# ReillyBova/Global-Illumination

Hardware: AMD Instinct MI355X
Metric: Mpixel-samples/sec (and ms/frame) at 1024^2 aa=2, 1M+1M photons (higher is better)
Workload: dtype f64 (shading/geometry), f32 (photon positions)

## Files before the change

### global-illumination_amd/csrc/gi_host.cpp

```cpp
#include <hip/hip_runtime.h>
#include <dlfcn.h>
#include <rccl/rccl.h>
#include <algorithm>
#include <cfloat>
#include <chrono>
#include <cmath>
#include <cstdio>
#include <cstdlib>
#include <cstring>
#include <functional>
#include <mutex>
#include <string>
#include <thread>
#include <vector>
#include "../../include/gi.h"
#include "gi_denoise.h"
#include "gi_radiance.h"
#include "gi_kdbuild.h"
#include "gi_kernels.h"
#include "gi_scene.h"
#include "gi_sort.h"

using namespace gi;

// ... 262 lines not shown
  DBuf d_nodes, d_elems, d_shapes, d_tris, d_bvh, d_mats, d_lights, d_lut, d_stats;
  HostMap hmap[2];
  DevMap dmap[2];
  bool map_valid[2] = {false, false};
  int leaf_size[2] = {64, 256};
  bool gpu_kd = true;
  KdBuildScratch kdb;
  DBuf kd_ph;
  int wave_cap_mul = 1;
  int chunk_cap_big = 512;
  bool chunk_dk_exact = true;
  int chunk_minsub_big = 64;
  int chunk_minsub = 32;
  double fb_ms[2] = {0, 0};
  uint64_t fb_q[2] = {0, 0};
  double p2_ms[2] = {0, 0};
  uint64_t p2_q[2] = {0, 0};
  int last_kind[2] = {-1, -1};
  bool knn_log = false;
  int knn_dbg = 0;
  int render_dbg = 0;
  int64_t slot_limit = 0;
  int elem_pretest = -1;
  gi_progress_fn progress = nullptr;
  void *progress_user = nullptr;
  int64_t progress_done = 0, progress_total = 0;
  int sel_slack = 64;
  int knn_qpl = 1;
  DBuf ind_cont, ind_ncont;
  DBuf mc_cont, mc_ncont;
  DBuf mc_cont2, mc_ncont2;
  bool mc_sub = true;
  int mc_persist = -1;
  DBuf prim_rgb;
  DBuf d_rays, d_ray_ids;
  std::vector<gi_ray> ray_stage;
  std::vector<uint64_t> id_stage;
  DBuf ind_tab, mc_tab;
  DBuf ind_trows, ind_rows;
  DBuf ind_masks;
  bool split_ind = true;
  double ind_frac = 0.25;
  DBuf spawn, npaths, path_off, nmc, mc_off, nind, ind_off, base, pixels, rgbf, rgb8, qcount, stats_bak;
  DBuf qpos[2], qshade[2], qkey[2], qout[2];
  bool chunk_big2 = true;
  int chunk_cap_big2 = 1024;
  int chunk_cap_big3 = 0;
  bool chunk_lane2 = true;
  int chunk_minsub_big2 = 64;
  bool chunk_dk = true;
  bool chunk_fb_all = false;
  int knn_general_mode = 0;
  int key_bits[2] = {10, 16};
  bool row_order = true;
  bool surf_key = true;
  bool surf_key_c = true;
  bool fb_wave = true;
  bool use_dk = true;
  DBuf qseg[2];
  size_t qcap_hint[2] = {0, 0};
  KeySortScratch keysort[2];
  int knn_kernel_kind = -1;
  DBuf scan_lvl[8], scan_out[8];
  DBuf pcounts, poffs, pbuf;
  DBuf pkeys, pcursor, ptmp;
  DBuf pacc, pglob;
// ... 918 lines not shown
    HIPCHK(c, c->ind_trows.ensure((size_t)(ntiles + 1) * 4));
    HIPCHK(c, c->ind_rows.ensure((size_t)(ntiles + 1) * 4));
    launch_ind_tiles(a.nind, nprim, c->ind_trows.as<uint32_t>(), c->stream);
    HIPCHK(c, launch_scan(c->ind_trows.as<uint32_t>(), c->ind_rows.as<uint32_t>(), ntiles, t, c->stream));
    uint32_t trows = 0;
    HIPCHK(c, hipMemcpyAsync(&trows, c->ind_rows.as<uint32_t>() + ntiles, 4, hipMemcpyDeviceToHost,
                             c->stream));
    HIPCHK(c, hipStreamSynchronize(c->stream));
    const uint64_t tind = 64ull * trows;
    if ((uint64_t)total_paths + tind + (uint64_t)nprim > slot_limit) {
      if (npix == 1)
        return fail(c, GI_ERR_ALLOC, "one output pixel's samples need more than 2^32 path slots");
      HIPCHK(c, hipMemcpyAsync(c->d_stats.p, c->stats_bak.p, ST_BYTES, hipMemcpyDeviceToDevice,
                               c->stream));
      HIPCHK(c, hipStreamSynchronize(c->stream));
      shrink *= 2;
      c->batch_reruns++;
      npix = 0;
      continue;
    }
    a.ind_rows = c->ind_rows.as<uint32_t>();
    a.ind_g0 = total_paths;
    a.tind = (int64_t)tind;
    HIPCHK(c, c->ind_tab.ensure(((size_t)trows + 1) * 8));
    launch_ind_row_tile(a.ind_rows, ntiles, c->ind_tab.as<uint64_t>(), c->stream);
    a.ind_row_info = c->ind_tab.as<uint64_t>();
    HIPCHK(c, c->ind_masks.ensure(((size_t)trows + 1) * 16));
    a.ind_qmask = c->ind_masks.as<uint64_t>();
    a.ind_bmask = a.ind_qmask + trows + 1;
    HIPCHK(c, c->base.ensure(((size_t)total_paths + tind) * 24));
    a.base = c->base.as<double>();
    const uint64_t ind_full = 64 * ((((uint64_t)a.tind + 63) / 64 + IND_QS - 1) / IND_QS);
    if (a.split_ind && a.total_ind > 0) HIPCHK(c, c->ind_ncont.ensure(IND_QS * 32 * 4));
    if (a.split_ind && a.total_mc > 0 && a.F.indirect) {
      const uint64_t full = 64 * ((((uint64_t)a.total_mc + 63) / 64 + IND_QS - 1) / IND_QS);
      HIPCHK(c, c->mc_cont.ensure((size_t)IND_QS * full * sizeof(IndCont)));
      HIPCHK(c, c->mc_ncont.ensure(IND_QS * 32 * 4));
      a.mc_cont = c->mc_cont.as<IndCont>();
      a.mc_ncont = c->mc_ncont.as<uint32_t>();
      a.mc_cap_s = (uint32_t)full;
      if (c->mc_persist > 0 || (c->mc_persist < 0 && !a.S.hard_lights)) {
        a.mc_next = c->qcount.as<uint32_t>() + 2;
        a.mc_persist_blocks = c->mc_persist > 0 ? c->mc_persist : 1024;
      }
      if (c->mc_sub) {
        HIPCHK(c, c->mc_cont2.ensure((size_t)IND_QS * full * sizeof(IndCont)));
        HIPCHK(c, c->mc_ncont2.ensure(IND_QS * 32 * 4));
        a.mc_cont2 = c->mc_cont2.as<IndCont>();
        a.mc_ncont2 = c->mc_ncont2.as<uint32_t>();
      }
    }
    uint32_t nq[2] = {0, 0};
    HIPCHK(c, hipMemcpyAsync(c->stats_bak.p, c->d_stats.p, ST_BYTES,
                             hipMemcpyDeviceToDevice, c->stream));
    uint32_t qbase[2] = {(uint32_t)(nprim + tind), (uint32_t)nprim};
    a.qind_base = nprim;
    a.tiled_skip = c->row_order && c->key_bits[0] <= 10 && !P.irradiance_cache && a.ind_qmask &&
                   (a.total_ind > 0 || tind == 0);
    for (int attempt = 0; attempt < 3; attempt++) {
      for (int l = 0; l < 2; l++) {
        size_t cap = std::max<size_t>(c->qcap_hint[l], (size_t)qbase[l] + 1024);
        if (attempt == 0) {
          const double per_mc = std::max(2.0, c->mc_app_rate[l]);
          size_t pred = (size_t)qbase[l] + (size_t)(1.25 * per_mc * (double)a.total_mc) + 1024;
          cap = std::max(cap, std::min<size_t>(pred, 0xFFFFFFF0u));
        }
        HIPCHK(c, c->qpos[l].ensure(cap * 16));
        HIPCHK(c, c->qshade[l].ensure(cap * sizeof(QShade)));
        HIPCHK(c, c->qkey[l].ensure(cap * 8));
        a.qpos[l] = c->qpos[l].as<float4>();
        a.qshade[l] = c->qshade[l].as<QShade>();
        a.qkey[l] = c->qkey[l].as<uint64_t>();
        a.qcap[l] = (uint32_t)std::min<size_t>(cap, 0xFFFFFFF0u);
      }
      if (a.split_ind && a.total_ind > 0) {
        uint64_t cap_s = std::min<uint64_t>(ind_full, 64 * ((uint64_t)(ind_full * c->ind_frac) / 64 + 1));
        HIPCHK(c, c->ind_cont.ensure((size_t)IND_QS * cap_s * sizeof(IndCont)));
        a.ind_cap_s = (uint32_t)cap_s;
        a.ind_cont = c->ind_cont.as<IndCont>();
        a.ind_ncont = c->ind_ncont.as<uint32_t>();
      }
      a.qcount = c->qcount.as<uint32_t>();
      HIPCHK(c, hipMemcpyAsync(c->qcount.p, qbase, 8, hipMemcpyHostToDevice, c->stream));
      if (!a.tiled_skip && tind > (uint64_t)a.total_ind) launch_ind_pad(a, c->stream);
      launch_path(a, c->stream, c->stream2, c->ev_fork, c->ev_join, true);
      HIPCHK(c, hipGetLastError());
      HIPCHK(c, hipMemcpyAsync(nq, c->qcount.p, 8, hipMemcpyDeviceToHost, c->stream));
      uint32_t fills[IND_QS * 32];
      if (a.split_ind && a.total_ind > 0)
        HIPCHK(c, hipMemcpyAsync(fills, c->ind_ncont.p, sizeof fills, hipMemcpyDeviceToHost, c->stream));
      HIPCHK(c, hipStreamSynchronize(c->stream));
      attempts_used = attempt + 1;
      bool ok = nq[0] <= a.qcap[0] && nq[1] <= a.qcap[1];
      if (a.split_ind && a.total_ind > 0) {
        uint32_t mx = 0;
        for (int q = 0; q < IND_QS; q++) mx = std::max(mx, fills[q * 32]);
        c->ind_frac = std::max(c->ind_frac, std::min(1.0, 1.25 * mx / (double)ind_full));
        if (mx > a.ind_cap_s) ok = false;
      }
      for (int l = 0; l < 2; l++)
        c->qcap_hint[l] = std::max<size_t>(c->qcap_hint[l], (size_t)(nq[l] * 1.25) + 1024);
      c->q_per_prim = std::max(c->q_per_prim, (double)((uint64_t)nq[0] + nq[1]) / (double)nprim);
      if (a.total_mc > 0)
        for (int l = 0; l < 2; l++)
          c->mc_app_rate[l] = std::max(c->mc_app_rate[l], (double)(nq[l] - qbase[l]) / (double)a.total_mc);
      if (ok) break;
      if (attempt == 2) return fail(c, GI_ERR_ALLOC, "query list overflow");
      HIPCHK(c, hipMemcpyAsync(c->d_stats.p, c->stats_bak.p, ST_BYTES,
                               hipMemcpyDeviceToDevice, c->stream));
    }
    bool run[2] = {false, false};
    for (int l = 0; l < 2; l++) {
      a.nq[l] = nq[l];
      a.qapp[l] = qbase[l];
      a.qout[l] = nullptr;
      if (nq[l]) {
        HIPCHK(c, c->qout[l].ensure((size_t)nq[l] * 24));
        a.qout[l] = c->qout[l].as<double>();
// ... 146 lines not shown
    c->mx[m].st = c->stream;
    hipEventCreate(&c->mx[m].ev0);
    hipEventCreate(&c->mx[m].ev1);
    hipEventCreate(&c->mx[m].ev2);
    hipEventCreate(&c->mx[m].ev3);
  }
  std::vector<double> lut;
  build_lut(lut);
  if (upload(c->d_lut, lut.data(), lut.size() * 8, c->stream) != hipSuccess ||
      c->d_stats.ensure(ST_BYTES) != hipSuccess) {
    delete c;
    return GI_ERR_HIP;
  }
  hipStreamSynchronize(c->stream);
  c->batch_log = (log_bits() & 2) != 0;
  c->knn_log = (log_bits() & 4) != 0;
  c->knn_dbg = (int)env_num("GI_KNN_DBG", 0);
  c->render_dbg = (int)env_num("GI_DBG", 0);
  c->slot_limit = (int64_t)env_num("GI_SLOT_LIMIT", 0);
  if (const int ls = (int)env_num("GI_LEAF_SIZE", 0); ls > 0) c->leaf_size[0] = c->leaf_size[1] = ls;
  c->gpu_kd = env_num("GI_HOST_KD", 0) == 0;
  c->photon_2pass = env_num("GI_PHOTON_2PASS", c->photon_2pass) != 0;
  c->prate[0] = c->prate[1] = std::max(0.0, env_num("GI_PHOTON_RATE0", c->prate[0]));
  c->chunk_minsub_big = std::min(64, std::max(1, (int)env_num("GI_CHUNK_MINSUB_BIG", c->chunk_minsub_big)));
  c->chunk_dk_exact = env_num("GI_CHUNK_DK_EXACT", c->chunk_dk_exact) != 0;
  c->chunk_cap_big3 = (int)env_num("GI_CHUNK_CAP_BIG3", c->chunk_cap_big3);
  c->chunk_minsub = std::min(64, std::max(1, (int)env_num("GI_CHUNK_MINSUB", c->chunk_minsub)));
  c->split_ind = env_num("GI_SPLIT_IND", c->split_ind) != 0;
  c->knn_general_mode = std::max(-1, std::min(1, (int)env_num("GI_KNN_GENERAL", c->knn_general_mode)));
  c->use_dk = env_num("GI_KNN_DK", c->use_dk) != 0;
  c->chunk_dk = env_num("GI_CHUNK_DK", c->chunk_dk) != 0;
  c->mc_sub = env_num("GI_MC_SUB", c->mc_sub) != 0;
  c->mc_persist = std::max(-1, (int)env_num("GI_MC_PERSIST", c->mc_persist));
  c->elem_pretest = env_num("GI_ELEM_PRETEST", c->elem_pretest) != 0;
  c->chunk_fb_all = env_num("GI_CHUNK_FB_ALL", c->chunk_fb_all) != 0;
  c->ind_frac = std::min(1.0, std::max(1e-6, env_num("GI_IND_FRAC", c->ind_frac)));
  c->knn_kernel_kind = (int)env_num("GI_KNN_KERNEL", c->knn_kernel_kind);
  c->row_order = env_num("GI_ROW_ORDER", c->row_order) != 0;
  c->surf_key = env_num("GI_SURF_KEY", c->surf_key) != 0;
  c->surf_key_c = env_num("GI_SURF_KEY_C", c->surf_key_c) != 0;
  c->fb_wave = env_num("GI_FB_WAVE", c->fb_wave) != 0;
  *out = c;
  return GI_OK;
}

int gi_create_devices(gi_ctx **out, const gi_device_set *set) {
  if (!out || !set || set->count < 1 || set->count > GI_MAX_DEVICES) return GI_ERR_ARG;
  *out = nullptr;
  gi_ctx *c = nullptr;
  int rc = gi_create(&c, set->devices[0]);
  if (rc) return rc;
  bool distinct = true;
  for (int k = 1; k < set->count; k++) {
    gi_ctx *d = nullptr;
    rc = gi_create(&d, set->devices[k]);
    if (rc) {
      gi_destroy(c);
      return rc;
    }
    c->peers.push_back(d);
    for (int j = 0; j < k; j++) distinct = distinct && set->devices[j] != set->devices[k];
  }
  if (set->count > 1 && distinct) {
    if (!g_rccl.load()) {
      gi_destroy(c);
      return GI_ERR_UNSUPPORTED;
// ... 28 lines not shown
      int r = -1;
      if (k < (int)c->comms.size() && c->comms[k] && g_rccl.commUserRank &&
          g_rccl.commUserRank(c->comms[k], &r) != ncclSuccess)
        r = -1;
      comm_rank[k] = r;
    }
  }
  if (comm_count) {
    int n = 0;
    if (!c->comms.empty() && c->comms[0] && g_rccl.commCount &&
        g_rccl.commCount(c->comms[0], &n) != ncclSuccess)
      n = 0;
    *comm_count = n;
  }
  return GI_OK;
}

struct DeviceScope {
  int prev = -1;
  explicit DeviceScope(int d) {
    if (hipGetDevice(&prev) != hipSuccess) prev = -1;
    hipSetDevice(d);
  }
  ~DeviceScope() {
    if (prev >= 0) hipSetDevice(prev);
  }
};

static void release_scratch(gi_ctx *c) {
  DBuf *bufs[] = {&c->spawn, &c->npaths, &c->path_off, &c->nmc, &c->mc_off, &c->nind,
                  &c->ind_off, &c->base, &c->pixels, &c->rgbf, &c->rgb8, &c->stats_bak,
                  &c->pcounts, &c->poffs, &c->pbuf, &c->pkeys, &c->pcursor, &c->ptmp, &c->pacc,
                  &c->pglob, &c->ind_cont, &c->ind_ncont, &c->mc_cont, &c->mc_ncont,
                  &c->mc_cont2, &c->mc_ncont2, &c->prim_rgb, &c->ind_tab, &c->mc_tab,
                  &c->ind_trows, &c->ind_rows, &c->ind_masks, &c->pack, &c->d_rays, &c->d_ray_ids,
                  &c->feat_samples, &c->feat_planes, &c->dn_rgbf, &c->dn_planes, &c->dn_img[0],
                  &c->dn_img[1], &c->rad_frame, &c->rad_samples, &c->rad_mean, &c->rad_var,
                  &c->acc_part, &c->tile_err, &c->tile_nmin, &c->tile_mask, &c->tm_in, &c->tm_out};
  for (DBuf *b : bufs) b->release();
  std::vector<gi_ray>().swap(c->ray_stage);
  std::vector<uint64_t>().swap(c->id_stage);
  for (auto &b : c->recv) b.release();
  for (auto &b : c->peer_pix) b.release();
  for (int m = 0; m < 2; m++) {
    MapExec &X = c->mx[m];
    DBuf *xb[] = {&X.list_idx, &X.list_d2, &X.list_n, &X.gheap_d2, &X.gheap_idx, &X.fb[0].list,
                  &X.fb[0].count, &X.fb[0].dense, &X.fb[1].list, &X.fb[1].count, &X.fb[1].dense,
                  &X.dk_q};
    for (DBuf *b : xb) b->release();
    sort_scratch_release(X.sorter);
  }
  for (int l = 0; l < 2; l++) {
    c->qpos[l].release(); c->qshade[l].release(); c->qkey[l].release(); c->qout[l].release();
    c->qseg[l].release();
    sort_scratch_release(c->keysort[l]);
  }
  sort_scratch_release(c->psort);
  for (int l = 0; l < 8; l++) { c->scan_lvl[l].release(); c->scan_out[l].release(); }
  c->kdb.release();
  c->kd_ph.release();
}

int gi_release_scratch(gi_ctx *c) {
  if (!c) return GI_ERR_ARG;
  DeviceScope scope(c->device);
  for (gi_ctx *d : c->peers) {
    hipSetDevice(d->device);
// ... 1632 lines not shown
```

### global-illumination_amd/csrc/gi_kernels.h

```cpp
#pragma once
#include <hip/hip_runtime.h>
#include <stdint.h>
#include "gi_device.h"

namespace gi {

struct gi_photon_dev {
  float pos[3];
  uint32_t rgbe;
  uint16_t dir;
  uint16_t flags;
};
static_assert(sizeof(gi_photon_dev) == 20, "photon record is 20 bytes");

struct gi_ray_dev {
  double org[3], dir[3];
};
static_assert(sizeof(gi_ray_dev) == 48, "ray record is 48 bytes");

struct Spawn {
  double p[3], n[3], v[3];
  double ct, R;
  double base[3];
  int32_t mat, hit;
  int32_t n_t, n_s, n_i;
  int32_t q_glob, q_caus;
  int32_t tri;
  double wt[3];
  uint64_t ind_key;
  double perp[3];
};
static_assert(sizeof(Spawn) == 200, "spawn record is 200 bytes");

struct IndCont {
  double org[3];
  double hp[3], hn[3];
  double w[3];
  uint64_t rkey, rctr;
  uint32_t g, prim;
  uint32_t pslot, qslot;
  int32_t mat;
  uint32_t j;
  int32_t tri;
  int32_t sub;
};

constexpr int IND_QS = 64;
constexpr uint32_t IND_EMPTY = 0xffffffffu;
constexpr int FB_QS = 64;

struct QShade {
  double n[3];
  double ex[3];
  double w[3];
};

enum {
  ST_RAY = 0, ST_SHADOW, ST_MONTE, ST_TRANS, ST_SPEC, ST_INDIRECT, ST_CAUSTIC,
  ST_KNN, ST_KNN_PHOTONS, ST_KNN_VISITED,
  ST_KNN_C, ST_KNN_C_PHOTONS, ST_KNN_C_VISITED,
  ST_GEN_MISS,
  ST_PHASE = 16,
  ST_COUNT = 32
};
enum { ST_KNN_MAP = ST_KNN_C - ST_KNN
};

struct RenderArgs {
  SceneView S;
  Flags F;
  const int2 *pixels;
  int32_t npix;
  int32_t af;
  int32_t W, H;
  int32_t dof_test;
  int32_t out_w;
  int64_t nprim;
  int64_t total_paths;
  Spawn *spawn;
  uint32_t *npaths;
  uint32_t *nmc;
  uint32_t *nind;
// ... 211 lines not shown
  int64_t e0;
  int64_t n;
  uint32_t *counts;
  const uint32_t *offsets;
  gi_photon_dev *out;
  uint32_t *cursor;
  uint64_t *keys;
  uint32_t cap;
  int32_t obits;
};
enum { PM_COUNT = 0, PM_EMIT = 1, PM_APPEND = 2 };

struct CameraRaysArgs {
  DCamera cam;
  uint64_t seed;
  int32_t dof, dof_test;
  int32_t af, W, H, out_w;
  int64_t first, n;
  gi_ray_dev *rays;
  uint64_t *ids;
};

struct ScanTemp {
  uint32_t *level[8];
  uint32_t *level_out[8];
  int depth;
};

hipError_t launch_scan(const uint32_t *in, uint32_t *out, int64_t n, ScanTemp &tmp,
                       hipStream_t st);
void launch_primary(const RenderArgs &a, hipStream_t st);
void launch_camera_rays(const CameraRaysArgs &a, hipStream_t st);
void launch_path(const RenderArgs &a, hipStream_t st, hipStream_t st2 = nullptr,
                 hipEvent_t fork = nullptr, hipEvent_t join = nullptr, bool wait_join = true);
void launch_photon_queries(const float *pos4, int64_t n, float4 *q, hipStream_t st);
void launch_fb_compact(const uint32_t *list, const uint32_t *count, uint32_t cap_s, uint32_t *dense,
                       uint32_t *total, hipStream_t st);
void launch_reduce(const RenderArgs &a, hipStream_t st);
void launch_owner_table(const uint32_t *off, int64_t n, uint32_t *tab, hipStream_t st);
void launch_ind_tiles(const uint32_t *nind, int64_t nprim, uint32_t *rows, hipStream_t st);
void launch_ind_row_tile(const uint32_t *rows, int64_t ntiles, uint64_t *tab, hipStream_t st);
void launch_ind_pad(const RenderArgs &a, hipStream_t st);
void launch_pack_pixels(const int32_t *pix_xy, int64_t n, int w, const float *rgbf,
                        const uint8_t *rgb8, void *out, hipStream_t st);
void launch_unpack_pixels(const int32_t *pix_xy, int64_t n, int w, const void *in, float *rgbf,
                          uint8_t *rgb8, hipStream_t st);
void launch_segments(const uint64_t *skeys, uint32_t n, uint32_t nprim, uint32_t *seg,
                     hipStream_t st);
void launch_knn(const KnnArgs &a, hipStream_t st);
bool launch_knn_wave(const KnnArgs &a, int cap_mul, hipStream_t st);
bool launch_knn_lane(const KnnArgs &a, hipStream_t st);
bool launch_knn_chunk(const KnnArgs &a, hipStream_t st);
bool launch_knn_chunk2(const KnnArgs &a, hipStream_t st);
bool launch_knn_chunk_big(const KnnArgs &a, int cap, hipStream_t st);
unsigned knn_chunk_grid(int64_t nq);
void launch_list_estimate(const KnnArgs &a, hipStream_t st);
void launch_cached(const KnnArgs &a, hipStream_t st);
void launch_photons(const PhotonArgs &a, int mode, hipStream_t st);
void launch_photon_gather(const gi_photon_dev *src, const uint32_t *slot, int64_t n,
                          gi_photon_dev *dst, hipStream_t st);
void launch_photon_rescale(gi_photon_dev *ph, int64_t n, double pp, hipStream_t st);
void launch_math_probe(int fn, int64_t n, const double *x, const double *y, double *out,
                       hipStream_t st);
void launch_intersect(const SceneView &S, int64_t n, const double *org, const double *dir,
                      int32_t *hit, double *t, double *point, double *normal, int32_t *mat,
                      hipStream_t st);

// ... 2 lines not shown
```

### global-illumination_amd/csrc/gi_kernels.hip

```cpp
#include <hip/hip_runtime.h>
#include "gi_device.h"
#include "gi_kernels.h"

namespace gi {

constexpr int SCAN_BLOCK = 256, SCAN_ITEMS = 4, SCAN_TILE = SCAN_BLOCK * SCAN_ITEMS;

__global__ __launch_bounds__(SCAN_BLOCK) void scan_tile_kernel(const uint32_t *in, uint32_t *out,
                                                                uint32_t *block_sums, int64_t n) {
  __shared__ uint32_t s[SCAN_BLOCK];
  int64_t base = (int64_t)blockIdx.x * SCAN_TILE + threadIdx.x * SCAN_ITEMS;
  uint32_t v[SCAN_ITEMS];
  uint32_t sum = 0;
#pragma unroll
  for (int i = 0; i < SCAN_ITEMS; i++) {
    int64_t k = base + i;
    v[i] = (k < n) ? in[k] : 0u;
    sum += v[i];
  }
  s[threadIdx.x] = sum;
  __syncthreads();
  for (int off = 1; off < SCAN_BLOCK; off <<= 1) {
    uint32_t t = (threadIdx.x >= (unsigned)off) ? s[threadIdx.x - off] : 0u;
    __syncthreads();
// ... 288 lines not shown
  org = h.p + sb * kEps;
  dir = sb;
  return true;
}

__device__ __forceinline__ bool diffuse_only(const DMaterial &m) {
  return !(m.flags & MF_TRANSPARENT) && m.max_kt == 0.0 && m.max_ks == 0.0;
}

template <uint32_t KINDS = KINDS_ALL>
__device__ __forceinline__ bool ind_bounce(PathCtx &P, V &org, V &dir, Rng &rng, C3 W, C3 &tw) {
  Hit h;
  if (!scene_intersect<KINDS>(*P.S, org, dir, h, P.hint)) {
    P.base += W * (tw * ldc(P.S->background));
    return false;
  }
  P.cnt.monte++;
  P.hint = h.tri;
  return ind_shade<false>(P, h, org, dir, rng, W, tw);
}

template <uint32_t KINDS = KINDS_ALL>
__device__ __forceinline__ void mc_indirect_body(PathCtx &P, V org, V dir, Rng &rng, C3 W) {
  C3 tw = rgb(1, 1, 1);
  for (int iter = 0; iter < P.F->max_monte_depth; iter++)
    if (!ind_bounce<KINDS>(P, org, dir, rng, W, tw)) break;
}

template <uint32_t KINDS = KINDS_ALL>
__device__ __noinline__ void mc_indirect(PathCtx &P, V org, V dir, Rng &rng, C3 W) {
  mc_indirect_body<KINDS>(P, org, dir, rng, W);
}

struct McLoop {
  V org, dir, ray_start;
  C3 tw, W;
  Rng rng;
  int iter;
};

__device__ __forceinline__ void mc_begin(McLoop &L, V org, V dir, const Rng &rng, C3 W) {
  L.org = org;
  L.dir = dir;
  L.ray_start = org;
  L.tw = rgb(1, 1, 1);
  L.W = W;
  L.rng = rng;
  L.iter = 0;
}

template <uint32_t KINDS = KINDS_ALL, bool DEFER = false, bool HARD = false>
__device__ __forceinline__ bool mc_step(PathCtx &P, McLoop &L) {
  const SceneView &S = *P.S;
  const Flags &F = *P.F;
  if (L.iter >= F.max_monte_depth) return false;
  L.iter++;
  const C3 W = L.W;
  Rng &rng = L.rng;
  C3 &tw = L.tw;
  Hit h;
  if (!scene_intersect<KINDS>(S, L.org, L.dir, h, P.hint)) {
    P.base += W * (tw * ldc(S.background));
    return false;
  }
  P.cnt.monte++;
  P.hint = h.tri;
  const DMaterial &m = S.mats[h.mat];
  C3 cb = rgb(0, 0, 0);
  if (F.ambient) cb += ldc(S.ambient);
  V view = normalize(h.p - L.ray_start);
  double ct = dot(h.n, -view);
  if (m.flags & (MF_DIFFUSE | MF_SPECULAR)) {
    if (HARD) direct_illumination_hard<KINDS>(S, F, h.p, h.n, L.ray_start, cb, m, ct, true, P.cnt);
    else direct_illumination<KINDS>(S, F, h.p, h.n, L.ray_start, cb, m, ct, true, rng, P.cnt);
  }
  if (F.caustic && (m.flags & MF_DIFFUSE)) {
    V ex = reflective_bounce(h.n, view, ct);
    put_query(P, 1, h.p, h.n, ex, ct, h.mat, W * tw);
    P.cnt.caustic++;
  }
  P.base += W * (cb * tw);
  double R = 0;
  if (F.specular && F.transmissive && F.fresnel && (m.flags & MF_TRANSPARENT))
    R = reflection_coeff_nc(F.ir_air, ct, m.ir);
  double pd = m.max_kd, pt = m.max_kt;
  double ps = m.max_ks + R * pt;
  pt *= (1.0 - R);
  double pterm = m.max_e + F.prob_absorb;
  double ptot = pd + pt + ps + pterm;
  double rnd = rng.next();
  if (ptot > 1.0) rnd *= ptot;
  V sb;
  if (rnd < pd) {
    C3 kd = ldc(m.kd);
    if (F.indirect) {
      V s2 = diffuse_sample_call(h.n, ct, rng);
      C3 w2 = W * ((kd * kd * tw) / pd);
      if (DEFER) {
        V o2 = h.p + s2 * kEps;
        size_t e;
        if (P.cont_slot >= 0) {
          e = (size_t)P.cont_slot;
        } else {
          int lane = (int)(threadIdx.x & 63);
          uint64_t act = __ballot(1);
          int leader = __ffsll((long long)act) - 1;
          uint32_t qb = 0;
          if (lane == leader) qb = atomicAdd(&P.A->mc_ncont[P.qstripe * 32], (uint32_t)__popcll(act));
          qb = (uint32_t)__shfl((int)qb, leader, 64);
          e = (size_t)P.qstripe * P.A->mc_cap_s + qb + (uint32_t)__popcll(act & ((1ull << lane) - 1ull));
        }
        IndCont &q = P.A->mc_cont[e];
        q.org[0] = o2.x; q.org[1] = o2.y; q.org[2] = o2.z;
        q.hp[0] = s2.x; q.hp[1] = s2.y; q.hp[2] = s2.z;
        q.w[0] = w2.r; q.w[1] = w2.g; q.w[2] = w2.b;
        q.rkey = rng.key;
        q.rctr = rng.ctr;
        q.g = (uint32_t)P.g;
        q.prim = P.prim;
        q.pslot = P.pslot;
        q.qslot = P.fixed[0] >= 0 ? (uint32_t)P.fixed[0] : 0xffffffffu;
        q.mat = -1;
        q.j = P.j;
        q.tri = h.tri;
        q.sub = 0;
        P.fixed[0] = -2;
      } else {
        mc_indirect<KINDS>(P, h.p + s2 * kEps, s2, rng, w2);
      }
      P.cnt.indirect++;
    } else if (F.fast_global) {
      V ex = reflective_bounce(h.n, view, ct);
      global_query(P, h.p, h.n, ex, ct, h.mat, W * (kd * tw / pd));
      if (!F.cache) P.cnt.indirect++;
    }
// ... 510 lines not shown
        V sb;
        C3 w;
        if (s < sp.n_t) {
          rng.init(F.seed, KIND_TRANS, psample, (uint64_t)s);
          V ex = transmissive_bounce_nc(F.ir_air, n, view, ct, m.ir);
          sb = F.distrib_trans ? specular_sample_call(ex, m.n, ct, rng) : ex;
          w = ((1.0 - R) * ldc(m.kt)) / (double)sp.n_t;
          P.cnt.trans++;
        } else {
          s -= sp.n_t;
          rng.init(F.seed, KIND_SPEC, psample, (uint64_t)s);
          V ex = reflective_bounce(n, view, ct);
          sb = F.distrib_spec ? specular_sample_call(ex, m.n, ct, rng) : ex;
          w = (ldc(m.kt) * R + ldc(m.ks)) / (double)sp.n_s;
          P.cnt.spec++;
        }
        mc_begin(L, p + sb * kEps, sb, rng, w);
        if (!F.monte_carlo) L.iter = F.max_monte_depth;
        active = true;
      } else {
        more = false;
      }
    }
    if (!__any(active)) break;
    if (active && !mc_step<KINDS, DEFER, HARD>(P, L)) {
      if (DEFER && P.fixed[0] != -2) a.mc_cont[P.cont_slot].g = IND_EMPTY;
      a.base[3 * P.g] = P.base.r;
      a.base[3 * P.g + 1] = P.base.g;
      a.base[3 * P.g + 2] = P.base.b;
      cnt.shadow += P.cnt.shadow; cnt.monte += P.cnt.monte; cnt.trans += P.cnt.trans;
      cnt.spec += P.cnt.spec; cnt.indirect += P.cnt.indirect; cnt.caustic += P.cnt.caustic;
      active = false;
    }
  }
  path_stats(a, cnt);
}

struct HeapRef {
  float *d2;
  int32_t *idx;
  int stride;
};

__device__ __forceinline__ bool heap_less(float da, int ia, float db, int ib) {
  return da < db || (da == db && ia < ib);
}

__device__ __forceinline__ void heap_push(HeapRef h, int &size, float d, int id) {
  int c = size++;
  while (c > 0) {
    int p = (c - 1) >> 1;
    float pd = h.d2[p * h.stride];
    int pi = h.idx[p * h.stride];
    if (!heap_less(pd, pi, d, id)) break;
    h.d2[c * h.stride] = pd;
    h.idx[c * h.stride] = pi;
    c = p;
  }
  h.d2[c * h.stride] = d;
  h.idx[c * h.stride] = id;
}
__device__ __forceinline__ void heap_replace_top(HeapRef h, int size, float d, int id) {
  int c = 0;
  while (true) {
    int l = 2 * c + 1;
    if (l >= size) break;
// ... 754 lines not shown
  }
  return hipMemcpyAsync(out + n, sums, sizeof(uint32_t), hipMemcpyDeviceToDevice, st);
}

void launch_primary(const RenderArgs &a, hipStream_t st) {
  if (a.spp) primary_rays_kernel<<<nblk(a.nprim, 256), 256, 0, st>>>(a);
  else primary_kernel<<<nblk(a.nprim, 256), 256, 0, st>>>(a);
}
void launch_camera_rays(const CameraRaysArgs &a, hipStream_t st) {
  if (a.n > 0) camera_rays_kernel<<<nblk(a.n, 256), 256, 0, st>>>(a);
}
template <uint32_t KINDS, bool RAYS>
void launch_ind(const RenderArgs &a, unsigned g, hipStream_t st) {
  if (KINDS == KINDS_TRI_SPHERE) ind_kernel<4, true, KINDS, RAYS><<<g, 128, 0, st>>>(a);
  else ind_kernel<3, true, KINDS, RAYS><<<g, 128, 0, st>>>(a);
}
void launch_cont(const RenderArgs &a, const IndCont *q, const uint32_t *fill, uint32_t cap_s,
                 hipStream_t st) {
  if ((a.S.kinds & ~KINDS_TRI_SPHERE) == 0)
    ind_cont_kernel<KINDS_TRI_SPHERE><<<IND_QS * 32, 128, 0, st>>>(a, q, fill, cap_s);
  else if ((a.S.kinds & ~KINDS_POLY) == 0)
    ind_cont_kernel<KINDS_POLY><<<IND_QS * 32, 128, 0, st>>>(a, q, fill, cap_s);
  else
    ind_cont_kernel<KINDS_ALL><<<IND_QS * 32, 128, 0, st>>>(a, q, fill, cap_s);
}
static void launch_mc_sub(const RenderArgs &a, hipStream_t st) {
  if ((a.S.kinds & ~KINDS_TRI_SPHERE) == 0)
    mc_sub_kernel<KINDS_TRI_SPHERE><<<IND_QS * 32, 128, 0, st>>>(a, a.mc_cont, a.mc_ncont, a.mc_cap_s);
  else if ((a.S.kinds & ~KINDS_POLY) == 0)
    mc_sub_kernel<KINDS_POLY><<<IND_QS * 32, 128, 0, st>>>(a, a.mc_cont, a.mc_ncont, a.mc_cap_s);
  else
    mc_sub_kernel<KINDS_ALL><<<IND_QS * 32, 128, 0, st>>>(a, a.mc_cont, a.mc_ncont, a.mc_cap_s);
}
template <bool RAYS>
static void launch_path_t(const RenderArgs &a, hipStream_t st, hipStream_t st2, hipEvent_t fork,
                          hipEvent_t join, bool wait_join) {
  const bool side = st2 && fork && join && a.total_mc > 0;
  hipStream_t ms = side ? st2 : st;
  if (a.total_mc > 0 && a.mc_cont) {
    (void)hipMemsetAsync(a.mc_ncont, 0, IND_QS * 32 * sizeof(uint32_t), st);
    if (a.mc_next) (void)hipMemsetAsync(a.mc_next, 0, sizeof(uint32_t), st);
    if (a.mc_cont2) (void)hipMemsetAsync(a.mc_ncont2, 0, IND_QS * 32 * sizeof(uint32_t), st);
  }
  if (a.total_ind > 0 && a.split_ind)
    (void)hipMemsetAsync(a.ind_ncont, 0, IND_QS * 32 * sizeof(uint32_t), st);
  if (side) {
    (void)hipEventRecord(fork, st);
    (void)hipStreamWaitEvent(st2, fork, 0);
  }
  if (a.nprim > 0) slot0_kernel<<<nblk(a.nprim, 256), 256, 0, st>>>(a);
  if (a.total_mc > 0) {
    unsigned g = nblk(a.total_mc, 128);
    if (a.mc_cont && a.mc_next) {
      unsigned gp = std::min(g, (unsigned)(a.mc_persist_blocks > 0 ? a.mc_persist_blocks : 1024));
      if ((a.S.kinds & ~KINDS_TRI_SPHERE) == 0) {
        if (a.S.hard_lights) mc_persist_kernel<KINDS_TRI_SPHERE, true, true, RAYS><<<gp, 128, 0, ms>>>(a);
        else mc_persist_kernel<KINDS_TRI_SPHERE, true, false, RAYS><<<gp, 128, 0, ms>>>(a);
      } else if ((a.S.kinds & ~KINDS_POLY) == 0) {
        if (a.S.hard_lights) mc_persist_kernel<KINDS_POLY, true, true, RAYS><<<gp, 128, 0, ms>>>(a);
        else mc_persist_kernel<KINDS_POLY, true, false, RAYS><<<gp, 128, 0, ms>>>(a);
      } else {
        mc_persist_kernel<KINDS_ALL, true, false, RAYS><<<gp, 128, 0, ms>>>(a);
      }
    } else if (a.mc_cont) {
      if ((a.S.kinds & ~KINDS_TRI_SPHERE) == 0) {
        if (a.S.hard_lights) mc_kernel<KINDS_TRI_SPHERE, true, true, RAYS><<<g, 128, 0, ms>>>(a);
        else mc_kernel<KINDS_TRI_SPHERE, true, false, RAYS><<<g, 128, 0, ms>>>(a);
      } else if ((a.S.kinds & ~KINDS_POLY) == 0) {
        if (a.S.hard_lights) mc_kernel<KINDS_POLY, true, true, RAYS><<<g, 128, 0, ms>>>(a);
        else mc_kernel<KINDS_POLY, true, false, RAYS><<<g, 128, 0, ms>>>(a);
      } else {
        mc_kernel<KINDS_ALL, true, false, RAYS><<<g, 128, 0, ms>>>(a);
      }
    }
    if (a.mc_cont) {
      if (a.mc_cont2) {
        launch_mc_sub(a, ms);
        launch_cont(a, a.mc_cont2, a.mc_ncont2, a.mc_cap_s, ms);
      } else {
        launch_cont(a, a.mc_cont, a.mc_ncont, a.mc_cap_s, ms);
      }
    } else {
      mc_kernel<KINDS_ALL, false, false, RAYS><<<g, 128, 0, ms>>>(a);
    }
  }
  if (a.total_ind > 0) {
    unsigned g = nblk(a.tind, 128);
    if (!a.split_ind) ind_kernel<2, false, KINDS_ALL, RAYS><<<g, 128, 0, st>>>(a);
    else if ((a.S.kinds & ~KINDS_TRI_SPHERE) == 0) launch_ind<KINDS_TRI_SPHERE, RAYS>(a, g, st);
    else if ((a.S.kinds & ~KINDS_POLY) == 0) launch_ind<KINDS_POLY, RAYS>(a, g, st);
    else launch_ind<KINDS_ALL, RAYS>(a, g, st);
    if (a.split_ind) launch_cont(a, a.ind_cont, a.ind_ncont, a.ind_cap_s, st);
  }
  if (side) {
    (void)hipEventRecord(join, st2);
    if (wait_join) (void)hipStreamWaitEvent(st, join, 0);
  }
}
void launch_path(const RenderArgs &a, hipStream_t st, hipStream_t st2, hipEvent_t fork,
                 hipEvent_t join, bool wait_join) {
  if (a.spp) launch_path_t<true>(a, st, st2, fork, join, wait_join);
  else launch_path_t<false>(a, st, st2, fork, join, wait_join);
}
__global__ void pack_pixels_kernel(const int2 *pix, int64_t n, int w, const float *rgbf,
                                   const uint8_t *rgb8, uint4 *out) {
  int64_t i = (int64_t)blockIdx.x * blockDim.x + threadIdx.x;
  if (i >= n) return;
  int2 p = pix[i];
  size_t o = 3 * ((size_t)p.y * w + p.x);
  uint32_t b = (uint32_t)rgb8[o] | ((uint32_t)rgb8[o + 1] << 8) | ((uint32_t)rgb8[o + 2] << 16);
  out[i] = make_uint4(__float_as_uint(rgbf[o]), __float_as_uint(rgbf[o + 1]),
                      __float_as_uint(rgbf[o + 2]), b);
}
__global__ void unpack_pixels_kernel(const int2 *pix, int64_t n, int w, const uint4 *in,
                                     float *rgbf, uint8_t *rgb8) {
  int64_t i = (int64_t)blockIdx.x * blockDim.x + threadIdx.x;
  if (i >= n) return;
  int2 p = pix[i];
  size_t o = 3 * ((size_t)p.y * w + p.x);
  uint4 v = in[i];
  rgbf[o] = __uint_as_float(v.x);
  rgbf[o + 1] = __uint_as_float(v.y);
  rgbf[o + 2] = __uint_as_float(v.z);
  rgb8[o] = (uint8_t)(v.w & 255u);
  rgb8[o + 1] = (uint8_t)((v.w >> 8) & 255u);
  rgb8[o + 2] = (uint8_t)((v.w >> 16) & 255u);
}
void launch_pack_pixels(const int32_t *pix_xy, int64_t n, int w, const float *rgbf,
                        const uint8_t *rgb8, void *out, hipStream_t st) {
  if (n == 0) return;
  pack_pixels_kernel<<<nblk(n, 256), 256, 0, st>>>(reinterpret_cast<const int2 *>(pix_xy), n, w,
                                                   rgbf, rgb8, reinterpret_cast<uint4 *>(out));
}
void launch_unpack_pixels(const int32_t *pix_xy, int64_t n, int w, const void *in, float *rgbf,
                          uint8_t *rgb8, hipStream_t st) {
// ... 82 lines not shown
```

Before: 13.17.

## Add wavefront-style multi-round MC path kernels with compacted live lists

For hard-light tri/sphere scenes, Monte Carlo specular/transmissive paths now run as a begin kernel followed by several per-bounce step kernels. Live path state is saved to a global state array between launches, and a compacted list of survivors keeps waves full instead of leaving lanes idle on divergent path lengths. A final tail kernel finishes the remaining bounces in a loop. This trades extra global memory traffic for the ~208-byte state per path, plus extra launches, in exchange for better SIMD utilisation. Continuation appends also switch to a per-stripe grouped atomic allocator, because lanes in a wave may now belong to different stripes.

```diff
diff --git a/global-illumination_amd/csrc/gi_host.cpp b/global-illumination_amd/csrc/gi_host.cpp
--- a/global-illumination_amd/csrc/gi_host.cpp
+++ b/global-illumination_amd/csrc/gi_host.cpp
@@ -318,6 +318,8 @@
   DBuf mc_cont2, mc_ncont2;
   bool mc_sub = true;
   int mc_persist = -1;
+  int mc_wave = -1;
+  DBuf mc_wstate, mc_wlist, mc_wcount;
   DBuf prim_rgb;
   DBuf d_rays, d_ray_ids;
   std::vector<gi_ray> ray_stage;
@@ -1302,6 +1304,8 @@
     a.base = c->base.as<double>();
     const uint64_t ind_full = 64 * ((((uint64_t)a.tind + 63) / 64 + IND_QS - 1) / IND_QS);
     if (a.split_ind && a.total_ind > 0) HIPCHK(c, c->ind_ncont.ensure(IND_QS * 32 * 4));
+    McWave mwave;
+    memset(&mwave, 0, sizeof mwave);
     if (a.split_ind && a.total_mc > 0 && a.F.indirect) {
       const uint64_t full = 64 * ((((uint64_t)a.total_mc + 63) / 64 + IND_QS - 1) / IND_QS);
       HIPCHK(c, c->mc_cont.ensure((size_t)IND_QS * full * sizeof(IndCont)));
@@ -1309,7 +1313,18 @@
       a.mc_cont = c->mc_cont.as<IndCont>();
       a.mc_ncont = c->mc_ncont.as<uint32_t>();
       a.mc_cap_s = (uint32_t)full;
-      if (c->mc_persist > 0 || (c->mc_persist < 0 && !a.S.hard_lights)) {
+      const bool wave_class = a.S.hard_lights && (a.S.kinds & ~KINDS_TRI_SPHERE) == 0;
+      const int rounds = c->mc_persist > 0 ? 0 : c->mc_wave >= 0 ? c->mc_wave : wave_class ? 4 : 0;
+      if (rounds > 0) {
+        HIPCHK(c, c->mc_wstate.ensure((size_t)a.total_mc * sizeof(McState)));
+        HIPCHK(c, c->mc_wlist.ensure(2 * (size_t)a.total_mc * 4));
+        HIPCHK(c, c->mc_wcount.ensure(((size_t)MC_WAVE_MAX_ROUNDS + 1) * 4));
+        mwave.state = c->mc_wstate.as<McState>();
+        mwave.list[0] = c->mc_wlist.as<uint32_t>();
+        mwave.list[1] = mwave.list[0] + a.total_mc;
+        mwave.count = c->mc_wcount.as<uint32_t>();
+        mwave.rounds = rounds;
+      } else if (c->mc_persist > 0 || (c->mc_persist < 0 && !a.S.hard_lights)) {
         a.mc_next = c->qcount.as<uint32_t>() + 2;
         a.mc_persist_blocks = c->mc_persist > 0 ? c->mc_persist : 1024;
       }
@@ -1353,7 +1368,8 @@
       a.qcount = c->qcount.as<uint32_t>();
       HIPCHK(c, hipMemcpyAsync(c->qcount.p, qbase, 8, hipMemcpyHostToDevice, c->stream));
       if (!a.tiled_skip && tind > (uint64_t)a.total_ind) launch_ind_pad(a, c->stream);
-      launch_path(a, c->stream, c->stream2, c->ev_fork, c->ev_join, true);
+      launch_path(a, c->stream, c->stream2, c->ev_fork, c->ev_join, true,
+                  mwave.rounds > 0 ? &mwave : nullptr);
       HIPCHK(c, hipGetLastError());
       HIPCHK(c, hipMemcpyAsync(nq, c->qcount.p, 8, hipMemcpyDeviceToHost, c->stream));
       uint32_t fills[IND_QS * 32];
@@ -1566,6 +1582,7 @@
   c->chunk_dk = env_num("GI_CHUNK_DK", c->chunk_dk) != 0;
   c->mc_sub = env_num("GI_MC_SUB", c->mc_sub) != 0;
   c->mc_persist = std::max(-1, (int)env_num("GI_MC_PERSIST", c->mc_persist));
+  c->mc_wave = std::min(MC_WAVE_MAX_ROUNDS, std::max(-1, (int)env_num("GI_MC_WAVE", c->mc_wave)));
   c->elem_pretest = env_num("GI_ELEM_PRETEST", c->elem_pretest) != 0;
   c->chunk_fb_all = env_num("GI_CHUNK_FB_ALL", c->chunk_fb_all) != 0;
   c->ind_frac = std::min(1.0, std::max(1e-6, env_num("GI_IND_FRAC", c->ind_frac)));
@@ -1660,7 +1677,8 @@
                   &c->ind_off, &c->base, &c->pixels, &c->rgbf, &c->rgb8, &c->stats_bak,
                   &c->pcounts, &c->poffs, &c->pbuf, &c->pkeys, &c->pcursor, &c->ptmp, &c->pacc,
                   &c->pglob, &c->ind_cont, &c->ind_ncont, &c->mc_cont, &c->mc_ncont,
-                  &c->mc_cont2, &c->mc_ncont2, &c->prim_rgb, &c->ind_tab, &c->mc_tab,
+                  &c->mc_cont2, &c->mc_ncont2, &c->mc_wstate, &c->mc_wlist, &c->mc_wcount,
+                  &c->prim_rgb, &c->ind_tab, &c->mc_tab,
                   &c->ind_trows, &c->ind_rows, &c->ind_masks, &c->pack, &c->d_rays, &c->d_ray_ids,
                   &c->feat_samples, &c->feat_planes, &c->dn_rgbf, &c->dn_planes, &c->dn_img[0],
                   &c->dn_img[1], &c->rad_frame, &c->rad_samples, &c->rad_mean, &c->rad_var,
diff --git a/global-illumination_amd/csrc/gi_kernels.h b/global-illumination_amd/csrc/gi_kernels.h
--- a/global-illumination_amd/csrc/gi_kernels.h
+++ b/global-illumination_amd/csrc/gi_kernels.h
@@ -48,6 +48,28 @@
 constexpr int IND_QS = 64;
 constexpr uint32_t IND_EMPTY = 0xffffffffu;
 constexpr int FB_QS = 64;
+
+struct alignas(16) McState {
+  double org[3], dir[3], ray_start[3];
+  double tw[3], W[3];
+  double base[3];
+  uint64_t rkey, rctr;
+  int64_t fixed[2];
+  uint32_t g, prim;
+  uint32_t pslot, j;
+  int32_t iter, hint;
+  uint32_t pad[2];
+};
+static_assert(sizeof(McState) == 208 && alignof(McState) == 16,
+              "path state record is 13 16-byte words");
+
+struct McWave {
+  McState *state;
+  uint32_t *list[2];
+  uint32_t *count;
+  int32_t rounds;
+};
+constexpr int MC_WAVE_MAX_ROUNDS = 1024;
 
 struct QShade {
   double n[3];
@@ -325,7 +347,8 @@
 void launch_primary(const RenderArgs &a, hipStream_t st);
 void launch_camera_rays(const CameraRaysArgs &a, hipStream_t st);
 void launch_path(const RenderArgs &a, hipStream_t st, hipStream_t st2 = nullptr,
-                 hipEvent_t fork = nullptr, hipEvent_t join = nullptr, bool wait_join = true);
+                 hipEvent_t fork = nullptr, hipEvent_t join = nullptr, bool wait_join = true,
+                 const McWave *mw = nullptr);
 void launch_photon_queries(const float *pos4, int64_t n, float4 *q, hipStream_t st);
 void launch_fb_compact(const uint32_t *list, const uint32_t *count, uint32_t cap_s, uint32_t *dense,
                        uint32_t *total, hipStream_t st);
diff --git a/global-illumination_amd/csrc/gi_kernels.hip b/global-illumination_amd/csrc/gi_kernels.hip
--- a/global-illumination_amd/csrc/gi_kernels.hip
+++ b/global-illumination_amd/csrc/gi_kernels.hip
@@ -344,6 +344,34 @@
   mc_indirect_body<KINDS>(P, org, dir, rng, W);
 }
 
+__device__ __forceinline__ void wave_list_append(uint32_t *list, uint32_t *count, bool keep,
+                                                 uint32_t v) {
+  const uint64_t m = __ballot(keep);
+  if (m == 0) return;
+  const int lane = (int)(threadIdx.x & 63);
+  const int leader = __ffsll((long long)m) - 1;
+  uint32_t b = 0;
+  if (lane == leader) b = atomicAdd(count, (uint32_t)__popcll(m));
+  b = (uint32_t)__shfl((int)b, leader, 64);
+  if (keep) list[b + (uint32_t)__popcll(m & ((1ull << lane) - 1ull))] = v;
+}
+__device__ __forceinline__ uint32_t wave_stripe_append(uint32_t *fill, uint32_t stripe) {
+  const int lane = (int)(threadIdx.x & 63);
+  uint64_t rem = __ballot(1);
+  uint32_t idx = 0;
+  while (rem) {
+    const int leader = __ffsll((long long)rem) - 1;
+    const uint32_t ls = (uint32_t)__shfl((int)stripe, leader, 64);
+    const uint64_t grp = __ballot(stripe == ls) & rem;
+    uint32_t b = 0;
+    if (lane == leader) b = atomicAdd(&fill[ls * 32], (uint32_t)__popcll(grp));
+    b = (uint32_t)__shfl((int)b, leader, 64);
+    if (stripe == ls) idx = b + (uint32_t)__popcll(grp & ((1ull << lane) - 1ull));
+    rem &= ~grp;
+  }
+  return idx;
+}
+
 struct McLoop {
   V org, dir, ray_start;
   C3 tw, W;
@@ -361,7 +389,7 @@
   L.iter = 0;
 }
 
-template <uint32_t KINDS = KINDS_ALL, bool DEFER = false, bool HARD = false>
+template <uint32_t KINDS = KINDS_ALL, bool DEFER = false, bool HARD = false, bool MIXED = false>
 __device__ __forceinline__ bool mc_step(PathCtx &P, McLoop &L) {
   const SceneView &S = *P.S;
   const Flags &F = *P.F;
@@ -413,6 +441,9 @@
         size_t e;
         if (P.cont_slot >= 0) {
           e = (size_t)P.cont_slot;
+        } else if (MIXED) {
+          e = (size_t)P.qstripe * P.A->mc_cap_s +
+              wave_stripe_append(P.A->mc_ncont, P.qstripe);
         } else {
           int lane = (int)(threadIdx.x & 63);
           uint64_t act = __ballot(1);
@@ -989,6 +1020,150 @@
       cnt.spec += P.cnt.spec; cnt.indirect += P.cnt.indirect; cnt.caustic += P.cnt.caustic;
       active = false;
     }
+  }
+  path_stats(a, cnt);
+}
+
+#ifndef MC_WAVE_WPE
+#define MC_WAVE_WPE 2
+#endif
+#ifndef MC_WAVE_BEGIN_WPE
+#define MC_WAVE_BEGIN_WPE 3
+#endif
+__device__ __forceinline__ void mc_state_store(McState &s, const PathCtx &P, const McLoop &L) {
+  s.org[0] = L.org.x; s.org[1] = L.org.y; s.org[2] = L.org.z;
+  s.dir[0] = L.dir.x; s.dir[1] = L.dir.y; s.dir[2] = L.dir.z;
+  s.ray_start[0] = L.ray_start.x; s.ray_start[1] = L.ray_start.y; s.ray_start[2] = L.ray_start.z;
+  s.tw[0] = L.tw.r; s.tw[1] = L.tw.g; s.tw[2] = L.tw.b;
+  s.W[0] = L.W.r; s.W[1] = L.W.g; s.W[2] = L.W.b;
+  s.base[0] = P.base.r; s.base[1] = P.base.g; s.base[2] = P.base.b;
+  s.rkey = L.rng.key;
+  s.rctr = L.rng.ctr;
+  s.fixed[0] = P.fixed[0];
+  s.fixed[1] = P.fixed[1];
+  s.g = (uint32_t)P.g;
+  s.prim = P.prim;
+  s.pslot = P.pslot;
+  s.j = P.j;
+  s.iter = L.iter;
+  s.hint = P.hint;
+}
+__device__ __forceinline__ void mc_state_load(const McState &s, const RenderArgs &a, uint32_t t,
+                                              PathCtx &P, McLoop &L) {
+  path_init(P, a, (int64_t)s.g, (int64_t)s.prim, (int)s.pslot);
+  P.j = s.j;
+  P.base = ldc(s.base);
+  P.fixed[0] = s.fixed[0];
+  P.fixed[1] = s.fixed[1];
+  P.hint = s.hint;
+  P.qstripe = (t >> 6) & (IND_QS - 1);
+  L.org = ld3(s.org);
+  L.dir = ld3(s.dir);
+  L.ray_start = ld3(s.ray_start);
+  L.tw = ldc(s.tw);
+  L.W = ldc(s.W);
+  L.rng.key = s.rkey;
+  L.rng.ctr = s.rctr;
+  L.iter = s.iter;
+}
+__device__ __forceinline__ void counts_add(Counts &c, const Counts &d) {
+  c.shadow += d.shadow; c.monte += d.monte; c.trans += d.trans;
+  c.spec += d.spec; c.indirect += d.indirect; c.caustic += d.caustic;
+}
+
+template <uint32_t KINDS, bool HARD, bool RAYS>
+__global__ __launch_bounds__(128)
+__attribute__((amdgpu_waves_per_eu((HARD && KINDS == KINDS_TRI_SPHERE) ? MC_WAVE_BEGIN_WPE : MC_WPE)))
+void mc_wave_begin_kernel(RenderArgs a, McWave w) {
+  const int64_t t = (int64_t)blockIdx.x * blockDim.x + threadIdx.x;
+  Counts cnt = {0, 0, 0, 0, 0, 0};
+  bool alive = false;
+  if (t < a.total_mc) {
+    const SceneView &S = a.S;
+    const Flags &F = a.F;
+    int64_t pb = wave_owner(a.mc_off, a.nprim, t, a.total_mc, a.mc_tab);
+    int s = (int)(t - a.mc_off[pb]);
+    const Spawn &sp = a.spawn[pb];
+    int64_t g = (int64_t)a.path_off[pb] + 1 + s;
+    int pix, i, j, k;
+    uint64_t psample;
+    decode_primary<RAYS>(a, pb, pix, i, j, k, psample);
+    const DMaterial &m = S.mats[sp.mat];
+    V p = ld3(sp.p), n = ld3(sp.n), view = ld3(sp.v);
+    double ct = sp.ct, R = sp.R;
+    PathCtx P;
+    McLoop L;
+    path_init(P, a, g, pb, 1 + s);
+    P.hint = sp.tri;
+    Rng rng;
+    V sb;
+    C3 wt;
+    if (s < sp.n_t) {
+      rng.init(F.seed, KIND_TRANS, psample, (uint64_t)s);
+      V ex = transmissive_bounce_nc(F.ir_air, n, view, ct, m.ir);
+      sb = F.distrib_trans ? specular_sample_call(ex, m.n, ct, rng) : ex;
+      wt = ((1.0 - R) * ldc(m.kt)) / (double)sp.n_t;
+      P.cnt.trans++;
+    } else {
+      s -= sp.n_t;
+      rng.init(F.seed, KIND_SPEC, psample, (uint64_t)s);
+      V ex = reflective_bounce(n, view, ct);
+      sb = F.distrib_spec ? specular_sample_call(ex, m.n, ct, rng) : ex;
+      wt = (ldc(m.kt) * R + ldc(m.ks)) / (double)sp.n_s;
+      P.cnt.spec++;
+    }
+    mc_begin(L, p + sb * kEps, sb, rng, wt);
+    if (!F.monte_carlo) L.iter = F.max_monte_depth;
+    alive = mc_step<KINDS, true, HARD>(P, L);
+    if (alive) {
+      mc_state_store(w.state[t], P, L);
+    } else {
+      a.base[3 * g] = P.base.r;
+      a.base[3 * g + 1] = P.base.g;
+      a.base[3 * g + 2] = P.base.b;
+    }
+    cnt = P.cnt;
+  }
+  wave_list_append(w.list[0], w.count, alive, (uint32_t)t);
+  path_stats(a, cnt);
+}
+
+template <uint32_t KINDS, bool HARD, bool TAIL>
+__global__ __launch_bounds__(128) __attribute__((amdgpu_waves_per_eu(MC_WAVE_WPE)))
+void mc_wave_step_kernel(RenderArgs a, McState *state, const uint32_t *in_list,
+                         const uint32_t *in_count, uint32_t *out_list, uint32_t *out_count,
+                         int steps) {
+  const int lane = (int)(threadIdx.x & 63);
+  const int64_t n = min((int64_t)*in_count, a.total_mc);
+  const int64_t stride = (int64_t)gridDim.x * blockDim.x;
+  int64_t i0 = (int64_t)blockIdx.x * blockDim.x + threadIdx.x - lane;
+  if (i0 >= n) return;
+  Counts cnt = {0, 0, 0, 0, 0, 0};
+  for (; i0 < n; i0 += stride) {
+    const int64_t i = i0 + lane;
+    bool alive = false;
+    uint32_t t = 0;
+    if (i < n) {
+      t = in_list[i];
+      PathCtx P;
+      McLoop L;
+      mc_state_load(state[t], a, t, P, L);
+      alive = true;
+      if (TAIL) {
+        for (int s = 0; s < steps && alive; s++) alive = mc_step<KINDS, true, HARD, true>(P, L);
+      } else {
+        alive = mc_step<KINDS, true, HARD, true>(P, L);
+      }
+      if (alive) {
+        mc_state_store(state[t], P, L);
+      } else {
+        a.base[3 * P.g] = P.base.r;
+        a.base[3 * P.g + 1] = P.base.g;
+        a.base[3 * P.g + 2] = P.base.b;
+      }
+      counts_add(cnt, P.cnt);
+    }
+    wave_list_append(out_list, out_count, alive, t);
   }
   path_stats(a, cnt);
 }
@@ -1809,11 +1984,25 @@
   else
     mc_sub_kernel<KINDS_ALL><<<IND_QS * 32, 128, 0, st>>>(a, a.mc_cont, a.mc_ncont, a.mc_cap_s);
 }
+template <uint32_t KINDS, bool HARD, bool RAYS>
+static void launch_mc_wave(const RenderArgs &a, const McWave &w, hipStream_t ms) {
+  const unsigned g = nblk(a.total_mc, 128);
+  mc_wave_begin_kernel<KINDS, HARD, RAYS><<<g, 128, 0, ms>>>(a, w);
+  for (int k = 1; k < w.rounds; k++)
+    mc_wave_step_kernel<KINDS, HARD, false><<<g, 128, 0, ms>>>(
+        a, w.state, w.list[(k - 1) & 1], w.count + (k - 1), w.list[k & 1], w.count + k, 1);
+  const int k = w.rounds;
+  mc_wave_step_kernel<KINDS, HARD, true><<<g, 128, 0, ms>>>(
+      a, w.state, w.list[(k - 1) & 1], w.count + (k - 1), w.list[k & 1], w.count + k,
+      std::max(1, a.F.max_monte_depth));
+}
 template <bool RAYS>
 static void launch_path_t(const RenderArgs &a, hipStream_t st, hipStream_t st2, hipEvent_t fork,
-                          hipEvent_t join, bool wait_join) {
+                          hipEvent_t join, bool wait_join, const McWave *mw) {
   const bool side = st2 && fork && join && a.total_mc > 0;
   hipStream_t ms = side ? st2 : st;
+  const bool wave = mw && mw->rounds > 0 && a.total_mc > 0 && a.mc_cont && !a.mc_next;
+  if (wave) (void)hipMemsetAsync(mw->count, 0, ((size_t)mw->rounds + 1) * sizeof(uint32_t), st);
   if (a.total_mc > 0 && a.mc_cont) {
     (void)hipMemsetAsync(a.mc_ncont, 0, IND_QS * 32 * sizeof(uint32_t), st);
     if (a.mc_next) (void)hipMemsetAsync(a.mc_next, 0, sizeof(uint32_t), st);
@@ -1839,6 +2028,16 @@
       } else {
         mc_persist_kernel<KINDS_ALL, true, false, RAYS><<<gp, 128, 0, ms>>>(a);
       }
+    } else if (wave) {
+      if ((a.S.kinds & ~KINDS_TRI_SPHERE) == 0) {
+        if (a.S.hard_lights) launch_mc_wave<KINDS_TRI_SPHERE, true, RAYS>(a, *mw, ms);
+        else launch_mc_wave<KINDS_TRI_SPHERE, false, RAYS>(a, *mw, ms);
+      } else if ((a.S.kinds & ~KINDS_POLY) == 0) {
+        if (a.S.hard_lights) launch_mc_wave<KINDS_POLY, true, RAYS>(a, *mw, ms);
+        else launch_mc_wave<KINDS_POLY, false, RAYS>(a, *mw, ms);
+      } else {
+        launch_mc_wave<KINDS_ALL, false, RAYS>(a, *mw, ms);
+      }
     } else if (a.mc_cont) {
       if ((a.S.kinds & ~KINDS_TRI_SPHERE) == 0) {
         if (a.S.hard_lights) mc_kernel<KINDS_TRI_SPHERE, true, true, RAYS><<<g, 128, 0, ms>>>(a);
@@ -1875,9 +2074,9 @@
   }
 }
 void launch_path(const RenderArgs &a, hipStream_t st, hipStream_t st2, hipEvent_t fork,
-                 hipEvent_t join, bool wait_join) {
-  if (a.spp) launch_path_t<true>(a, st, st2, fork, join, wait_join);
-  else launch_path_t<false>(a, st, st2, fork, join, wait_join);
+                 hipEvent_t join, bool wait_join, const McWave *mw) {
+  if (a.spp) launch_path_t<true>(a, st, st2, fork, join, wait_join, mw);
+  else launch_path_t<false>(a, st, st2, fork, join, wait_join, mw);
 }
 __global__ void pack_pixels_kernel(const int2 *pix, int64_t n, int w, const float *rgbf,
                                    const uint8_t *rgb8, uint4 *out) {
```

New measurement: 13.43 (median of 6 runs). 1.02x the previous value.
